# facebookresearch/vilbert-multi-task

Measured on AMD Instinct MI355X. Metric: samples/sec (36 regions, 36 tokens) ViLBERT-base 6L/6C fwd+bwd, higher is better.
Workload: dtype f32; 1 GPU; bert_base_6layer_6conect.json train_concap step: BertForMultiModalPreTraining fwd+bwd (dropout on) + grad all-reduce + AdamW, 36 regions + 1 global row, batch 256 per GPU, T=36 R=37; per_gpu_batch=256, global_batch=256, parallelism=dp1, visible_gpus=1, launch=eager, gemm_mode=f32, deterministic_wgrad=True, deterministic_fallbacks=0

## Files before the change

### vilbert-multi-task_amd/csrc/common.h

```cpp
#pragma once
#include <hip/hip_runtime.h>
#include <stdint.h>

#include "bf16_round.h"
#include "gemm_plan.h"

typedef float f32x4 __attribute__((ext_vector_type(4)));
typedef float f32x16 __attribute__((ext_vector_type(16)));

#define VB_LAUNCH_CHECK()                         \
    do {                                          \
        hipError_t e__ = hipGetLastError();       \
        if (e__ != hipSuccess) return (int)e__;   \
    } while (0)

const uint64_t* vb_seed_epoch();

namespace vbemb {
int text_embed_bwd_det(hipStream_t st, int batch, int n_tok, int hidden, int vocab, int n_types, int n_tasks,
                       const int64_t* ids, const int64_t* seg, const int64_t* task_ids, const float* dx, float* dword,
                       float* dpos, float* dtype, float* dtask);
}

namespace vbrows {
int gather(hipStream_t st, long M, int cols, const float* src, const int32_t* map, long src_rows, float* out);
int drop_add(hipStream_t st, long M, int cols, const float* lin, const float* res, bool res_mapped, const int32_t* map,
             long src_rows, float* out, float p, uint64_t seed);
int invert(hipStream_t st, long src_rows, long M, const int32_t* map, int32_t* inv);
int scatter(hipStream_t st, long src_rows, int cols, const float* compact, const int32_t* inv, float* full);
int scatter_stats(hipStream_t st, long src_rows, const float* v0, const float* v1, const float* v2, const float* v3,
                  const int32_t* inv, float* full);
}

__device__ __forceinline__ float wave_sum(float v) {
#pragma unroll
    for (int off = 32; off > 0; off >>= 1) v += __shfl_xor(v, off, 64);
    return v;
}

__device__ __forceinline__ void gelu_parts(float x, float& phi, float& e) {
    const float z = fabsf(x) * 0.70710678118654752440f;
    const float t = __builtin_amdgcn_rcpf(fmaf(0.3275911f, z, 1.0f));
    e = __expf(-z * z);
    float poly = fmaf(1.061405429f, t, -1.453152027f);
    poly = fmaf(poly, t, 1.421413741f);
    poly = fmaf(poly, t, -0.284496736f);
    poly = fmaf(poly, t, 0.254829592f);
    const float half_erfc = 0.5f * poly * t * e;
    phi = x >= 0.f ? 1.0f - half_erfc : half_erfc;
}

__device__ __forceinline__ float gelu_erf(float x) {
    float phi, e;
    gelu_parts(x, phi, e);
    return x * phi;
}

__device__ __forceinline__ float gelu_grad(float x) {
    float phi, e;
    gelu_parts(x, phi, e);
    return fmaf(x * 0.39894228040143267794f, e, phi);
}

__device__ __forceinline__ void gelu_and_grad(float x, float& y, float& d) {
    float phi, e;
    gelu_parts(x, phi, e);
    y = x * phi;
    d = fmaf(x * 0.39894228040143267794f, e, phi);
}

__device__ __forceinline__ float swish_act(float x) {
    return x / (1.0f + expf(-x));
}

__device__ __forceinline__ float swish_grad(float x) {
    const float s = 1.0f / (1.0f + expf(-x));
    return s + x * s * (1.0f - s);
}
```

### vilbert-multi-task_amd/csrc/layers.hip

```cpp
#include "common.h"
#include "row_map.h"
#include <mutex>
#include <unordered_map>

namespace {

constexpr bool kF32 = false, kB16 = true;

#define VB_TRY(expr)               \
    do {                           \
        const int _e = (expr);     \
        if (_e != 0) return _e;    \
    } while (0)

template <bool B16>
struct Elem { static constexpr size_t size = B16 ? 2 : 4; };

template <bool B16>
inline const void* col(const void* p, long c) { return static_cast<const char*>(p) + c * (long)Elem<B16>::size; }
template <bool B16>
inline void* col(void* p, long c) { return static_cast<char*>(p) + c * (long)Elem<B16>::size; }

bool has_bias(const vb_layer_linear& L) { return L.bias[0] != nullptr; }
bool wants_wgrad(const vb_layer_linear& L) { return L.dw[0] != nullptr; }
// ... 121 lines not shown
        a.mask_add = c.mask; a.O = static_cast<uint16_t*>(c.out); a.ldo = c.ldo; a.lse = c.lse;
        a.scale = scale; a.dropout_p = c.p; a.seed = c.seed;
        return vb_attention_fwd_bf16(st, &a);
    }
    vb_attention_args a{};
    a.batch = c.batch; a.heads = c.heads; a.head_dim = c.d; a.n_q = c.n_q; a.n_k = c.n_k;
    a.q_batch = c.batch; a.kv_batch = c.batch;
    a.Q = static_cast<const float*>(c.q); a.ldq = c.ldq;
    a.K = static_cast<const float*>(c.k); a.ldk = c.ldk;
    a.V = static_cast<const float*>(c.v); a.ldv = c.ldk;
    a.mask_add = c.mask; a.O = static_cast<float*>(c.out); a.ldo = c.ldo; a.lse = c.lse;
    a.scale = scale; a.dropout_p = c.p; a.seed = c.seed;
    return vb_attention_fwd(st, &a);
}

template <bool B16>
int attn_bwd(void* st, const AttnCall& c, const void* d_out, void* dq, void* dk, void* dv, long lddq, long lddk, float* dvec) {
    const float scale = (float)(1.0 / sqrt((double)c.d));
    if (B16) {
        vb_attention_bf16_args a{};
        a.batch = c.batch; a.heads = c.heads; a.head_dim = c.d; a.n_q = c.n_q; a.n_k = c.n_k;
        a.q_batch = c.batch; a.kv_batch = c.batch;
        a.Q = static_cast<const uint16_t*>(c.q); a.ldq = c.ldq;
        a.K = static_cast<const uint16_t*>(c.k); a.ldk = c.ldk;
        a.V = static_cast<const uint16_t*>(c.v); a.ldv = c.ldk;
        a.mask_add = c.mask; a.lse = c.lse; a.scale = scale; a.dropout_p = c.p; a.seed = c.seed;
        vb_attention_bf16_grads g{};
        g.dO = static_cast<const uint16_t*>(d_out); g.lddo = c.ldo;
        g.dQ = static_cast<uint16_t*>(dq); g.lddq = lddq;
        g.dK = static_cast<uint16_t*>(dk); g.lddk = lddk;
        g.dV = static_cast<uint16_t*>(dv); g.lddv = lddk;
        g.dvec = dvec;
        return vb_attention_bwd_bf16(st, &a, &g);
    }
    vb_attention_args a{};
    a.batch = c.batch; a.heads = c.heads; a.head_dim = c.d; a.n_q = c.n_q; a.n_k = c.n_k;
    a.q_batch = c.batch; a.kv_batch = c.batch;
    a.Q = static_cast<const float*>(c.q); a.ldq = c.ldq;
    a.K = static_cast<const float*>(c.k); a.ldk = c.ldk;
    a.V = static_cast<const float*>(c.v); a.ldv = c.ldk;
    a.mask_add = c.mask; a.lse = c.lse; a.scale = scale; a.dropout_p = c.p; a.seed = c.seed;
    vb_attention_grads g{};
    g.dO = static_cast<const float*>(d_out); g.lddo = c.ldo;
    g.dQ = static_cast<float*>(dq); g.lddq = lddq;
    g.dK = static_cast<float*>(dk); g.lddk = lddk;
    g.dV = static_cast<float*>(dv); g.lddv = lddk;
    g.dvec = dvec;
    return vb_attention_bwd(st, &a, &g);
}

std::mutex g_ev_mutex;
std::unordered_map<void*, hipEvent_t> g_fork_events;

int fork_to(void* main_st, void* side_st) {
    hipEvent_t ev;
    {
        std::lock_guard<std::mutex> lock(g_ev_mutex);
        auto it = g_fork_events.find(main_st);
        if (it == g_fork_events.end()) {
            const hipError_t e = hipEventCreateWithFlags(&ev, hipEventDisableTiming);
            if (e != hipSuccess) return (int)e;
            g_fork_events.emplace(main_st, ev);
        } else {
            ev = it->second;
        }
    }
    hipError_t e = hipEventRecord(ev, static_cast<hipStream_t>(main_st));
    if (e != hipSuccess) return (int)e;
    e = hipStreamWaitEvent(static_cast<hipStream_t>(side_st), ev, 0);
    return e == hipSuccess ? 0 : (int)e;
}

struct WgradJob { long M; const vb_layer_linear* L; const void* dY; const void* X; };
struct WgradQueue {
    WgradJob job[8];
    int n = 0;
    void push(long M, const vb_layer_linear& L, const void* dY, const void* X) {
        if (wants_wgrad(L) && n < 8) job[n++] = WgradJob{M, &L, dY, X};
    }
};

template <bool B16>
int wgrad_flush(void* st, void* side, const WgradQueue& q) {
    if (q.n == 0) return 0;
    void* target = st;
    if (side != nullptr && side != st) {
        VB_TRY(fork_to(st, side));
        target = side;
    }
    for (int i = 0; i < q.n; ++i) VB_TRY(wgrad<B16>(target, q.job[i].M, *q.job[i].L, q.job[i].dY, q.job[i].X));
    return 0;
}

AttnCall self_call(const vb_attn_block& b, bool b16) {
    const long Hb = (long)b.heads * b.head_dim, es = b16 ? 2 : 4;
    AttnCall c{};
    c.batch = b.batch; c.heads = b.heads; c.d = b.head_dim; c.n_q = b.n1; c.n_k = b.n1;
    c.q = b.qkv1_out;
    c.k = static_cast<const char*>(b.qkv1_out) + Hb * es;
    c.v = static_cast<const char*>(b.qkv1_out) + 2 * Hb * es;
    c.ldq = c.ldk = 3 * Hb;
    c.mask = b.mask1; c.out = b.ctx1; c.ldo = Hb; c.lse = b.lse1; c.p = b.p1; c.seed = b.seed1;
    return c;
}
AttnCall cross_call(const vb_attn_block& b, bool b16, int which) {
    const long Hb = (long)b.heads * b.head_dim, es = b16 ? 2 : 4;
    const void* qsrc = which == 1 ? b.qkv2_out : b.qkv1_out;
    const void* ksrc = which == 1 ? b.qkv1_out : b.qkv2_out;
    AttnCall c{};
    c.batch = b.batch; c.heads = b.heads; c.d = b.head_dim;
    c.n_q = which == 1 ? b.n2 : b.n1;
    c.n_k = which == 1 ? b.n1 : b.n2;
    c.q = qsrc;
    c.k = static_cast<const char*>(ksrc) + Hb * es;
    c.v = static_cast<const char*>(ksrc) + 2 * Hb * es;
    c.ldq = c.ldk = 3 * Hb;
    c.mask = which == 1 ? b.mask1 : b.mask2;
    c.out = which == 1 ? b.ctx1 : b.ctx2;
    c.ldo = Hb;
    c.lse = which == 1 ? b.lse1 : b.lse2;
    c.p = which == 1 ? b.p1 : b.p2;
    c.seed = which == 1 ? b.seed1 : b.seed2;
    return c;
}

template <bool B16>
int attn_block_fwd(void* st, const vb_attn_block& b) {
    const long M1 = (long)b.batch * b.n1;
    VB_TRY(linear<B16>(st, M1, b.qkv1, b.x1, b.qkv1_out, VB_ACT_NONE, nullptr, 0.f, 0, nullptr));
    if (b.n2 == 0) return attn_fwd<B16>(st, self_call(b, B16));
    const long M2 = (long)b.batch * b.n2;
    VB_TRY(linear<B16>(st, M2, b.qkv2, b.x2, b.qkv2_out, VB_ACT_NONE, nullptr, 0.f, 0, nullptr));
    VB_TRY(attn_fwd<B16>(st, cross_call(b, B16, 1)));
    return attn_fwd<B16>(st, cross_call(b, B16, 2));
}

int ffn_block_rows_fwd(void* st, const vb_ffn_block& f, bool training) {
    hipStream_t hs = static_cast<hipStream_t>(st);
    const long M = f.M, R = f.src_rows;
    float *sum1 = static_cast<float*>(f.sum1), *sum2 = static_cast<float*>(f.sum2);
    VB_TRY(vbrows::gather(hs, M, f.Hc, static_cast<const float*>(f.ctx), f.row_map, R, static_cast<float*>(f.ctx_rows)));
    VB_TRY(linear<kF32>(st, M, f.o, f.ctx_rows, sum1, VB_ACT_NONE, nullptr, 0.f, 0, nullptr));
    VB_TRY(vbrows::drop_add(hs, M, f.H, sum1, static_cast<const float*>(f.x), true, f.row_map, R, sum1, f.p_o, f.seed_o));
    VB_TRY(ln_fwd<kF32>(st, M, f.H, sum1, f.ln1, f.eps, f.a1, training ? f.mean1 : nullptr, training ? f.rstd1 : nullptr));
    VB_TRY(linear<kF32>(st, M, f.f1, f.a1, f.h, VB_ACT_GELU, nullptr, 0.f, 0, training ? f.dact : nullptr));
    VB_TRY(linear<kF32>(st, M, f.f2, f.h, sum2, VB_ACT_NONE, nullptr, 0.f, 0, nullptr));
    VB_TRY(vbrows::drop_add(hs, M, f.H, sum2, static_cast<const float*>(f.a1), false, f.row_map, R, sum2, f.p_f, f.seed_f));
    return ln_fwd<kF32>(st, M, f.H, sum2, f.ln2, f.eps, f.y, training ? f.mean2 : nullptr, training ? f.rstd2 : nullptr);
}

int ffn_block_rows_bwd(void* st, WgradQueue& wq, const vb_ffn_block& f) {
    hipStream_t hs = static_cast<hipStream_t>(st);
    const long M = f.M, R = f.src_rows;
    const vbrows::FullWs w(R, f.H, f.I);
    float* ws = f.full_ws;
    int32_t* inv = reinterpret_cast<int32_t*>(ws + w.inv);
    float* stats = ws + w.stats;
    auto compact = [](const void* p) { return static_cast<const float*>(p); };
    VB_TRY(vbrows::invert(hs, R, M, f.row_map, inv));
    VB_TRY(vbrows::scatter_stats(hs, R, f.mean1, f.rstd1, f.mean2, f.rstd2, inv, stats));
    VB_TRY(vbrows::scatter(hs, R, f.H, compact(f.dy), inv, ws + w.dy));
    VB_TRY(vbrows::scatter(hs, R, f.H, compact(f.sum2), inv, ws + w.sum2));
    VB_TRY(ln_bwd<kF32>(st, R, f.H, ws + w.dy, ws + w.sum2, stats + 2 * R, stats + 3 * R, f.ln2, ws + w.d_sum2, f.ln_ws,
                        ws + w.d_sum2_drop, f.p_f, f.seed_f));
    const float* dyd_full = f.p_f > 0.f ? ws + w.d_sum2_drop : ws + w.d_sum2;
    VB_TRY(vbrows::gather(hs, M, f.H, ws + w.d_sum2, f.row_map, R, static_cast<float*>(f.d_sum2)));
    const void* dyd = f.d_sum2;
    if (f.p_f > 0.f) {
        VB_TRY(vbrows::gather(hs, M, f.H, dyd_full, f.row_map, R, static_cast<float*>(f.d_sum2_drop)));
        dyd = f.d_sum2_drop;
    }
    VB_TRY(dgrad<kF32>(st, M, f.f2, dyd, f.d_pre, nullptr, f.dact));
    VB_TRY(vbrows::scatter(hs, R, f.I, compact(f.h), inv, ws + w.h));
    wq.push(R, f.f2, dyd_full, ws + w.h);
    VB_TRY(dgrad<kF32>(st, M, f.f1, f.d_pre, f.d_a1, f.d_sum2, nullptr));
    VB_TRY(vbrows::scatter(hs, R, f.I, compact(f.d_pre), inv, ws + w.d_pre));
    VB_TRY(vbrows::scatter(hs, R, f.H, compact(f.a1), inv, ws + w.a1));
    wq.push(R, f.f1, ws + w.d_pre, ws + w.a1);
    VB_TRY(vbrows::scatter(hs, R, f.H, compact(f.d_a1), inv, ws + w.d_a1));
    VB_TRY(vbrows::scatter(hs, R, f.H, compact(f.sum1), inv, ws + w.sum1));
    VB_TRY(ln_bwd<kF32>(st, R, f.H, ws + w.d_a1, ws + w.sum1, stats, stats + R, f.ln1, f.d_sum1_full, f.ln_ws,
                        ws + w.d_sum1_drop, f.p_o, f.seed_o));
    const float* dod_full = f.p_o > 0.f ? ws + w.d_sum1_drop : static_cast<const float*>(f.d_sum1_full);
    float* dod = static_cast<float*>(f.p_o > 0.f ? f.d_sum1_drop : f.d_sum1);
    VB_TRY(vbrows::gather(hs, M, f.H, dod_full, f.row_map, R, dod));
    VB_TRY(dgrad<kF32>(st, M, f.o, dod, f.d_ctx, nullptr, nullptr));
    wq.push(R, f.o, dod_full, f.ctx);
    return vbrows::scatter(hs, R, f.Hc, compact(f.d_ctx), inv, static_cast<float*>(f.d_ctx_full));
}

template <bool B16>
int ffn_block_fwd(void* st, const vb_ffn_block& f, bool training) {
    if (f.M == 0) return 0;
    if (f.row_map != nullptr) return ffn_block_rows_fwd(st, f, training);
    VB_TRY(linear<B16>(st, f.M, f.o, f.ctx, f.sum1, VB_ACT_NONE, f.x, f.p_o, f.seed_o, nullptr));
    VB_TRY(ln_fwd<B16>(st, f.M, f.H, f.sum1, f.ln1, f.eps, f.a1, training ? f.mean1 : nullptr, training ? f.rstd1 : nullptr));
    VB_TRY(linear<B16>(st, f.M, f.f1, f.a1, f.h, VB_ACT_GELU, nullptr, 0.f, 0, training ? f.dact : nullptr));
    VB_TRY(linear<B16>(st, f.M, f.f2, f.h, f.sum2, VB_ACT_NONE, f.a1, f.p_f, f.seed_f, nullptr));
    return ln_fwd<B16>(st, f.M, f.H, f.sum2, f.ln2, f.eps, f.y, training ? f.mean2 : nullptr, training ? f.rstd2 : nullptr);
}

template <bool B16>
int ffn_block_bwd(void* st, WgradQueue& wq, const vb_ffn_block& f) {
    if (f.M == 0) return 0;
    if (f.row_map != nullptr) return ffn_block_rows_bwd(st, wq, f);
    VB_TRY(ln_bwd<B16>(st, f.M, f.H, f.dy, f.sum2, f.mean2, f.rstd2, f.ln2, f.d_sum2, f.ln_ws, f.d_sum2_drop, f.p_f, f.seed_f));
    const void* dyd = f.p_f > 0.f ? f.d_sum2_drop : f.d_sum2;
    VB_TRY(dgrad<B16>(st, f.M, f.f2, dyd, f.d_pre, nullptr, f.dact));
    wq.push(f.M, f.f2, dyd, f.h);
    VB_TRY(dgrad<B16>(st, f.M, f.f1, f.d_pre, f.d_a1, f.d_sum2, nullptr));
    wq.push(f.M, f.f1, f.d_pre, f.a1);
    VB_TRY(ln_bwd<B16>(st, f.M, f.H, f.d_a1, f.sum1, f.mean1, f.rstd1, f.ln1, f.d_sum1, f.ln_ws, f.d_sum1_drop, f.p_o, f.seed_o));
    const void* dod = f.p_o > 0.f ? f.d_sum1_drop : f.d_sum1;
    VB_TRY(dgrad<B16>(st, f.M, f.o, dod, f.d_ctx, nullptr, nullptr));
    wq.push(f.M, f.o, dod, f.ctx);
    return 0;
}

template <bool B16>
int attn_block_bwd(void* st, WgradQueue& wq, const vb_attn_block& b) {
    const long Hb = (long)b.heads * b.head_dim, M1 = (long)b.batch * b.n1;
    if (b.n2 == 0) {
        VB_TRY(attn_bwd<B16>(st, self_call(b, B16), b.d_ctx1, b.dqkv1, col<B16>(b.dqkv1, Hb), col<B16>(b.dqkv1, 2 * Hb), 3 * Hb,
                             3 * Hb, b.dvec));
    } else {
        VB_TRY(attn_bwd<B16>(st, cross_call(b, B16, 1), b.d_ctx1, b.dqkv2, col<B16>(b.dqkv1, Hb), col<B16>(b.dqkv1, 2 * Hb), 3 * Hb,
                             3 * Hb, b.dvec));
        VB_TRY(attn_bwd<B16>(st, cross_call(b, B16, 2), b.d_ctx2, b.dqkv1, col<B16>(b.dqkv2, Hb), col<B16>(b.dqkv2, 2 * Hb), 3 * Hb,
                             3 * Hb, b.dvec));
    }
    if (b.dx1 != nullptr) VB_TRY(dgrad<B16>(st, M1, b.qkv1, b.dqkv1, b.dx1, b.dres1, nullptr));
    wq.push(M1, b.qkv1, b.dqkv1, b.x1);
    if (b.n2 != 0) {
        const long M2 = (long)b.batch * b.n2;
        if (b.dx2 != nullptr) VB_TRY(dgrad<B16>(st, M2, b.qkv2, b.dqkv2, b.dx2, b.dres2, nullptr));
        wq.push(M2, b.qkv2, b.dqkv2, b.x2);
    }
    return 0;
}

bool bad_linear(const vb_layer_linear& L, bool b16) {
    if (L.nseg < 1 || L.nseg > VB_MAX_SEGMENTS || L.seg_n <= 0 || L.K <= 0) return true;
    if (b16) return L.w16 == nullptr;
    for (int s = 0; s < L.nseg; ++s)
        if (L.w[s] == nullptr) return true;
    return false;
}

int check(const vb_layer_args* a, bool backward) {
    if (a == nullptr) return VB_E_BADARG;
    if (a->dtype != VB_DT_F32 && a->dtype != VB_DT_BF16) return VB_E_BADARG;
    const bool b16 = a->dtype == VB_DT_BF16;
    const vb_attn_block& b = a->attn;
    const bool has_attn = b.batch != 0;
    if (!has_attn && a->s1.M == 0 && a->s2.M == 0) return VB_E_BADARG;
    if (has_attn) {
        if (b.batch < 0 || b.heads <= 0 || b.head_dim <= 0 || b.n1 <= 0 || b.n2 < 0) return VB_E_BADARG;
        if (b.x1 == nullptr || b.qkv1_out == nullptr || b.ctx1 == nullptr || bad_linear(b.qkv1, b16)) return VB_E_BADARG;
        if ((long)b.qkv1.nseg * b.qkv1.seg_n != 3L * b.heads * b.head_dim) return VB_E_SEGMENT;
        if (b.n2 > 0) {
            if (b.x2 == nullptr || b.qkv2_out == nullptr || b.ctx2 == nullptr || bad_linear(b.qkv2, b16)) return VB_E_BADARG;
            if ((long)b.qkv2.nseg * b.qkv2.seg_n != 3L * b.heads * b.head_dim) return VB_E_SEGMENT;
        }
    }
    for (const vb_ffn_block* f : {&a->s1, &a->s2}) {
        if (f->M == 0) continue;
        if (f->M < 0 || f->H <= 0 || f->I <= 0 || f->Hc <= 0) return VB_E_BADARG;
        if (bad_linear(f->o, b16) || bad_linear(f->f1, b16) || bad_linear(f->f2, b16)) return VB_E_BADARG;
        if (f->o.K != f->Hc || f->o.nseg * f->o.seg_n != f->H || f->f1.K != f->H || f->f1.nseg * f->f1.seg_n != f->I ||
            f->f2.K != f->I || f->f2.nseg * f->f2.seg_n != f->H)
            return VB_E_SEGMENT;
        if (f->ctx == nullptr || f->x == nullptr || f->sum1 == nullptr || f->a1 == nullptr || f->h == nullptr || f->sum2 == nullptr ||
            f->y == nullptr || f->ln1.gamma == nullptr || f->ln2.gamma == nullptr)
            return VB_E_BADARG;
        if (backward) {
            if (f->dy == nullptr || f->d_sum2 == nullptr || f->d_pre == nullptr || f->d_a1 == nullptr || f->d_sum1 == nullptr ||
                f->d_ctx == nullptr || f->ln_ws == nullptr || f->dact == nullptr || f->mean1 == nullptr || f->mean2 == nullptr ||
                f->ln1.dgamma == nullptr || f->ln2.dgamma == nullptr)
                return VB_E_BADARG;
            if ((f->p_f > 0.f && f->d_sum2_drop == nullptr) || (f->p_o > 0.f && f->d_sum1_drop == nullptr)) return VB_E_BADARG;
        }
        if (int e = vbrows::check_row_map(*f, b16, backward)) return e;
    }
    if (backward && has_attn &&
        (b.dqkv1 == nullptr || b.dvec == nullptr || b.d_ctx1 == nullptr || b.lse1 == nullptr ||
         (b.n2 > 0 && (b.dqkv2 == nullptr || b.d_ctx2 == nullptr || b.lse2 == nullptr))))
        return VB_E_BADARG;
    return 0;
}

template <bool B16>
int layer_fwd(void* st, const vb_layer_args* a) {
    if (a->attn.batch != 0) VB_TRY(attn_block_fwd<B16>(st, a->attn));
    VB_TRY(ffn_block_fwd<B16>(st, a->s1, a->training != 0));
    return ffn_block_fwd<B16>(st, a->s2, a->training != 0);
}

template <bool B16>
int layer_bwd(void* st, const vb_layer_args* a) {
    static const bool each = [] { const char* e = getenv("VB_WGRAD_FORK"); return e != nullptr && e[0] == 'e'; }();
    WgradQueue wq;
    VB_TRY(ffn_block_bwd<B16>(st, wq, a->s1));
    if (each) { VB_TRY(wgrad_flush<B16>(st, a->wgrad_stream, wq)); wq.n = 0; }
    VB_TRY(ffn_block_bwd<B16>(st, wq, a->s2));
    if (each) { VB_TRY(wgrad_flush<B16>(st, a->wgrad_stream, wq)); wq.n = 0; }
    if (a->attn.batch != 0) VB_TRY(attn_block_bwd<B16>(st, wq, a->attn));
    return wgrad_flush<B16>(st, a->wgrad_stream, wq);
}

}

extern "C" int vb_layer_fwd(void* stream, const vb_layer_args* a) {
    VB_TRY(check(a, false));
    return a->dtype == VB_DT_BF16 ? layer_fwd<kB16>(stream, a) : layer_fwd<kF32>(stream, a);
}

extern "C" int vb_layer_bwd(void* stream, const vb_layer_args* a) {
    VB_TRY(check(a, true));
    return a->dtype == VB_DT_BF16 ? layer_bwd<kB16>(stream, a) : layer_bwd<kF32>(stream, a);
}
```

### vilbert-multi-task_amd/csrc/rowmap.hip

```cpp
#include "common.h"
#include "rng.h"
#include "row_map.h"

namespace {

__device__ __forceinline__ long source_row(const int32_t* __restrict__ map, long r, long src_rows) {
    const long s = map[r];
    return s >= 0 && s < src_rows ? s : -1;
}

__global__ __launch_bounds__(256) void gather_rows_kernel(long M, int cols4, const f32x4* __restrict__ src,
                                                          const int32_t* __restrict__ map, long src_rows,
                                                          f32x4* __restrict__ out) {
    const long n = M * cols4;
    for (long i = (long)blockIdx.x * blockDim.x + threadIdx.x; i < n; i += (long)gridDim.x * blockDim.x) {
        const long r = i / cols4, c = i - r * cols4;
        const long s = source_row(map, r, src_rows);
        out[i] = s >= 0 ? src[s * cols4 + c] : f32x4{0.f, 0.f, 0.f, 0.f};
    }
}

__global__ __launch_bounds__(256) void row_drop_add_kernel(long M, int cols4, const f32x4* lin, const f32x4* __restrict__ res,
                                                           int res_mapped, const int32_t* __restrict__ map, long src_rows,
                                                           f32x4* out, float p, float scale, uint64_t seed_in,
                                                           const uint64_t* __restrict__ epoch) {
    const uint64_t seed = p > 0.f ? vb_seed_with_epoch(seed_in, epoch) : 0;
    const long n = M * cols4;
    for (long i = (long)blockIdx.x * blockDim.x + threadIdx.x; i < n; i += (long)gridDim.x * blockDim.x) {
        const long r = i / cols4, c = i - r * cols4;
        const long s = source_row(map, r, src_rows);
        f32x4 o = {0.f, 0.f, 0.f, 0.f};
        if (s >= 0) {
            f32x4 v = lin[i];
            if (p > 0.f) {
                const uint64_t idx = (uint64_t)((s * cols4 + c) * 4);
#pragma unroll
                for (int e = 0; e < 4; ++e) v[e] = vb_keep(seed, idx + e, p) ? v[e] * scale : 0.f;
            }
            o = v;
            if (res != nullptr) o += res[(res_mapped ? s : r) * cols4 + c];
        }
        out[i] = o;
    }
}

__global__ __launch_bounds__(256) void invert_map_kernel(long src_rows, int M, const int32_t* __restrict__ map,
                                                         int32_t* __restrict__ inv) {
    const int lane = threadIdx.x & 63;
    const long R = (long)blockIdx.x * 4 + (threadIdx.x >> 6);
    if (R >= src_rows) return;
    int found = -1;
    for (int base = 0; base < M && found < 0; base += 64) {
        const int r = base + lane;
        const unsigned long long hits = __ballot(r < M && (long)map[r] == R);
        if (hits != 0) found = base + __ffsll(hits) - 1;
    }
    if (lane == 0) inv[R] = found;
}

__global__ __launch_bounds__(256) void scatter_rows_kernel(long src_rows, int cols4, const f32x4* __restrict__ compact,
                                                           const int32_t* __restrict__ inv, f32x4* __restrict__ full) {
    const long n = src_rows * cols4;
    for (long i = (long)blockIdx.x * blockDim.x + threadIdx.x; i < n; i += (long)gridDim.x * blockDim.x) {
        const long R = i / cols4, c = i - R * cols4;
        const long r = inv[R];
        full[i] = r >= 0 ? compact[r * cols4 + c] : f32x4{0.f, 0.f, 0.f, 0.f};
    }
}

__global__ __launch_bounds__(256) void scatter_stats_kernel(long src_rows, const float* __restrict__ v0, const float* __restrict__ v1,
                                                            const float* __restrict__ v2, const float* __restrict__ v3,
                                                            const int32_t* __restrict__ inv, float* __restrict__ full) {
    for (long R = (long)blockIdx.x * blockDim.x + threadIdx.x; R < src_rows; R += (long)gridDim.x * blockDim.x) {
        const long r = inv[R];
        full[R] = r >= 0 ? v0[r] : 0.f;
        full[src_rows + R] = r >= 0 ? v1[r] : 0.f;
        full[2 * src_rows + R] = r >= 0 ? v2[r] : 0.f;
        full[3 * src_rows + R] = r >= 0 ? v3[r] : 0.f;
    }
}

inline unsigned grid_for(long work_items) {
    long blocks = (work_items + 255) / 256;
    if (blocks > 2048) blocks = 2048;
    if (blocks < 1) blocks = 1;
    return (unsigned)blocks;
}

}

namespace vbrows {

int gather(hipStream_t st, long M, int cols, const float* src, const int32_t* map, long src_rows, float* out) {
    hipLaunchKernelGGL(gather_rows_kernel, dim3(grid_for(M * (cols / 4))), dim3(256), 0, st, M, cols / 4,
                       reinterpret_cast<const f32x4*>(src), map, src_rows, reinterpret_cast<f32x4*>(out));
    VB_LAUNCH_CHECK();
    return 0;
}

int drop_add(hipStream_t st, long M, int cols, const float* lin, const float* res, bool res_mapped, const int32_t* map,
             long src_rows, float* out, float p, uint64_t seed) {
    hipLaunchKernelGGL(row_drop_add_kernel, dim3(grid_for(M * (cols / 4))), dim3(256), 0, st, M, cols / 4,
                       reinterpret_cast<const f32x4*>(lin), reinterpret_cast<const f32x4*>(res), res_mapped ? 1 : 0, map, src_rows,
                       reinterpret_cast<f32x4*>(out), p, 1.0f / (1.0f - p), seed, p > 0.f ? vb_seed_epoch() : nullptr);
    VB_LAUNCH_CHECK();
    return 0;
}

int invert(hipStream_t st, long src_rows, long M, const int32_t* map, int32_t* inv) {
    hipLaunchKernelGGL(invert_map_kernel, dim3((unsigned)((src_rows + 3) / 4)), dim3(256), 0, st, src_rows, (int)M, map, inv);
    VB_LAUNCH_CHECK();
    return 0;
}

int scatter(hipStream_t st, long src_rows, int cols, const float* compact, const int32_t* inv, float* full) {
    hipLaunchKernelGGL(scatter_rows_kernel, dim3(grid_for(src_rows * (cols / 4))), dim3(256), 0, st, src_rows, cols / 4,
                       reinterpret_cast<const f32x4*>(compact), inv, reinterpret_cast<f32x4*>(full));
    VB_LAUNCH_CHECK();
    return 0;
}

int scatter_stats(hipStream_t st, long src_rows, const float* v0, const float* v1, const float* v2, const float* v3,
                  const int32_t* inv, float* full) {
    hipLaunchKernelGGL(scatter_stats_kernel, dim3(grid_for(src_rows)), dim3(256), 0, st, src_rows, v0, v1, v2, v3, inv, full);
    VB_LAUNCH_CHECK();
    return 0;
}

}
```

### vilbert-multi-task_amd/vilbert/layers.py

```python
import ctypes
import os
import weakref

import torch
from torch.autograd import Function

from . import _native as N
from . import arena as _arena
from . import autograd_ops as A
from . import ops
from . import ops16

BF16 = torch.bfloat16
_STATE = {"on": os.environ.get("VB_LAYER_NATIVE", "1") != "0", "calls": 0}


def set_native(on):
    prev, _STATE["on"] = _STATE["on"], bool(on)
    return prev


def native_calls():
    return _STATE["calls"]

# ... 150 lines not shown
    _static_linear(f.o, [p[0]], [p[1]])
    f.ln1.gamma, f.ln1.beta = p[2].data_ptr(), p[3].data_ptr()
    _static_linear(f.f1, [p[4]], [p[5]])
    _static_linear(f.f2, [p[6]], [p[7]])
    f.ln2.gamma, f.ln2.beta = p[8].data_ptr(), p[9].data_ptr()


def _dyn_ffn_fwd(f, c, base, ctx_ptr, x_ptr, y_ptr, p, dyn, b16, training):
    f.ctx, f.x, f.y = ctx_ptr, x_ptr, y_ptr
    f.p_o, f.p_f, f.seed_o, f.seed_f = dyn
    if b16:
        _shadow_linear(f.o, [p[0]])
        _shadow_linear(f.f1, [p[4]])
        _shadow_linear(f.f2, [p[6]])
    at = c.at
    f.sum1, f.a1, f.h, f.sum2 = at(base, "sum1"), at(base, "a1"), at(base, "h"), at(base, "sum2")
    if training:
        f.dact = at(base, "dact")
        f.mean1, f.rstd1, f.mean2, f.rstd2 = at(base, "mean1"), at(base, "rstd1"), at(base, "mean2"), at(base, "rstd2")


def _dyn_ffn_bwd(f, t, tbase, dy_ptr, d_sum1_ptr, d_ctx_ptr, tg, pbase, ws, dyn):
    p_o, p_f = dyn[0], dyn[1]
    at = t.at
    f.dy = dy_ptr
    f.d_sum2, f.d_pre, f.d_a1 = at(tbase, "d_sum2"), at(tbase, "d_pre"), at(tbase, "d_a1")
    f.d_sum2_drop = at(tbase, "d_sum2_drop") if p_f > 0.0 else None
    f.d_sum1_drop = at(tbase, "d_sum1_drop") if p_o > 0.0 else None
    f.d_sum1, f.d_ctx = d_sum1_ptr, d_ctx_ptr
    f.ln_ws = ws.data_ptr()
    _set_linear_targets(f.o, tg, [pbase + 0], [pbase + 1])
    f.ln1.dgamma, f.ln1.dbeta = tg.overwrite_target(pbase + 2), tg.overwrite_target(pbase + 3)
    _set_linear_targets(f.f1, tg, [pbase + 4], [pbase + 5])
    _set_linear_targets(f.f2, tg, [pbase + 6], [pbase + 7])
    f.ln2.dgamma, f.ln2.dbeta = tg.overwrite_target(pbase + 8), tg.overwrite_target(pbase + 9)


def _ffn_plan(p, dims, b16, training):
    plan = _Plan()
    plan.params, plan.b16, plan.training, plan.dims = list(p), b16, training, dims
    M, _Hc, H, I, _eps = dims
    es = 2 if b16 else 4
    plan.c_fwd = _Carver()
    _ffn_sizes(plan.c_fwd, M, H, I, es, training)
    plan.c_bwd = _Carver()
    _ffn_bwd_sizes(plan.c_bwd, M, H, I, es)
    a = N.LayerArgs()
    a.dtype, a.training = (1 if b16 else 0), int(training)
    _static_ffn(a.s1, p, dims)
    _seal(plan, a)
    return plan


class FfnBlockFn(Function):

    @staticmethod
    def forward(ctx, ctx_t, x, plan, dyn, *p):
        b16, training, c = plan.b16, plan.training, plan.c_fwd
        ctx_t, x = ops._contig(ctx_t), ops._contig(x)
        buf = c.alloc(x.device)
        y = torch.empty_like(x)
        a = plan.new_args()
        _dyn_ffn_fwd(a.s1, c, buf.data_ptr(), ctx_t.data_ptr(), x.data_ptr(), y.data_ptr(), p, dyn, b16, training)
        _call(N.lib().vb_layer_fwd, a, "vb_layer_fwd (output + FFN block)")
        if training:
            ctx.save_for_backward(ctx_t, x, buf, *p)
            ctx.plan, ctx.dyn = plan, dyn
        return y

    @staticmethod
    def backward(ctx, dy):
        ctx_t, x, buf = ctx.saved_tensors[:3]
        p = ctx.saved_tensors[3:]
        plan, dyn = ctx.plan, ctx.dyn
        b16, c, t = plan.b16, plan.c_fwd, plan.c_bwd
        M, _Hc, H, _I, _eps = plan.dims
        dy = ops._contig(dy)
        dev = x.device
        N.ensure_deterministic(dev)
        tg = _Targets(list(p), dev)
        side, ws_stream = _side_stream_for(dev, tg)
        tbuf = t.alloc(dev)
        d_x = torch.empty_like(x)
        d_ctx = torch.empty_like(ctx_t)
        a = plan.new_args()
        a.training, a.wgrad_stream = 1, side
        _dyn_ffn_fwd(a.s1, c, buf.data_ptr(), ctx_t.data_ptr(), x.data_ptr(), buf.data_ptr(), p, dyn, b16, True)
        _dyn_ffn_bwd(a.s1, t, tbuf.data_ptr(), dy.data_ptr(), d_x.data_ptr(), d_ctx.data_ptr(), tg, 0, _ln_ws(dev, M, H, b16), dyn)
        _call(N.lib().vb_layer_bwd, a, "vb_layer_bwd (output + FFN block)")
        if ws_stream is not None:
            for tt in (buf, tbuf, ctx_t, d_x):
                tt.record_stream(ws_stream)
            if dyn[0] == 0.0:
                A.hold_for_side_stream(ws_stream, d_x)
        grads = tg.finish()
        return (d_ctx, d_x, None, None) + tuple(grads)


def _static_attn(b, adims, p):
    b.batch, b.heads, b.head_dim, b.n1, b.n2 = adims
    _static_linear(b.qkv1, [p[0], p[2], p[4]], [p[1], p[3], p[5]])
    if adims[4]:
        _static_linear(b.qkv2, [p[6], p[8], p[10]], [p[7], p[9], p[11]])


def _dyn_attn_fwd(b, n2, x1, x2, mask1, mask2, qkv1, qkv2, ctx1, ctx2, lse1, lse2, p, adyn, b16):
    b.x1, b.mask1, b.qkv1_out, b.ctx1, b.lse1 = x1, mask1, qkv1, ctx1, lse1
    b.p1, b.p2, b.seed1, b.seed2 = adyn
    if b16:
        _shadow_linear(b.qkv1, [p[0], p[2], p[4]])
    if n2:
        b.x2, b.mask2, b.qkv2_out, b.ctx2, b.lse2 = x2, mask2, qkv2, ctx2, lse2
        if b16:
            _shadow_linear(b.qkv2, [p[6], p[8], p[10]])


def _mask2d(mask, B, S):
    if mask is None:
        return None
    m = ops._contig(mask)
    if m.numel() != B * S:
        raise RuntimeError("attention: mask must hold %d x %d values" % (B, S))
    N.dev_f32(m, "attention mask")
    return m


def _ptr(t):
    return t.data_ptr() if t is not None else None


def _self_plan(p, adims, dims, b16, training, row_cap=None):
    plan = _Plan()
    plan.params, plan.b16, plan.training = list(p), b16, training
    plan.dims, plan.row_cap = (adims, dims), row_cap
    B, heads, _d, S, _n2 = adims
    M, _Hc, H, I, _eps = dims
    Mb = M if row_cap is None else row_cap
    es = 2 if b16 else 4
    c = plan.c_fwd = _Carver()
    _ffn_sizes(c, Mb, H, I, es, training)
    c.add("qkv", M * 3 * H * es)
    c.add("ctx", M * H * es)
    if row_cap is not None:
        c.add("ctx_rows", Mb * H * es)
    if training:
        c.add("lse", B * heads * S * 4)
    t = plan.c_bwd = _Carver()
    _ffn_bwd_sizes(t, Mb, H, I, es)
    t.add("d_sum1", M * H * es)
    t.add("d_ctx", M * H * es)
    if row_cap is not None:
        t.add("d_sum1_rows", Mb * H * es)
        t.add("d_ctx_rows", Mb * H * es)
        t.add("full_ws", M * (8 * H + 2 * I + 5) * 4)
    t.add("dqkv", M * 3 * H * es)
    t.add("dvec", B * heads * S * 4)
    a = N.LayerArgs()
    a.dtype, a.training = (1 if b16 else 0), int(training)
    _static_attn(a.attn, adims, p)
    _static_ffn(a.s1, p[6:], dims)
    if row_cap is not None:
        a.s1.src_rows = M
    _seal(plan, a)
    return plan


class SelfLayerFn(Function):

    @staticmethod
    def forward(ctx, x, mask, rows, plan, dyn, *p):
        b16, training, c = plan.b16, plan.training, plan.c_fwd
        (B, _heads, _d, S, _n2), _dims = plan.dims
        x = ops._contig(x)
        mask = _mask2d(mask, B, S)
        buf = c.alloc(x.device)
        base = buf.data_ptr()
        y = torch.empty_like(x) if rows is None else torch.empty((rows.numel(), x.shape[-1]), dtype=x.dtype, device=x.device)
        a = plan.new_args()
        cx = c.at(base, "ctx")
        _dyn_attn_fwd(a.attn, 0, x.data_ptr(), None, _ptr(mask), None, c.at(base, "qkv"), None, cx, None,
                      c.at(base, "lse") if training else None, None, p, (dyn[4], 0.0, dyn[5], 0), b16)
        _dyn_ffn_fwd(a.s1, c, base, cx, x.data_ptr(), y.data_ptr(), p[6:], dyn[:4], b16, training)
        if rows is not None:
            a.s1.M, a.s1.row_map, a.s1.ctx_rows = rows.numel(), rows.data_ptr(), c.at(base, "ctx_rows")
        _call(N.lib().vb_layer_fwd, a, "vb_layer_fwd")
        if training:
            ctx.save_for_backward(x, mask, buf, rows, *p)
            ctx.plan, ctx.dyn = plan, dyn
        return y

    @staticmethod
    def backward(ctx, dy):
        x, mask, buf, rows = ctx.saved_tensors[:4]
        p = ctx.saved_tensors[4:]
        plan, dyn = ctx.plan, ctx.dyn
        b16, c, t = plan.b16, plan.c_fwd, plan.c_bwd
        _adims, (M, _Hc, H, _I, _eps) = plan.dims
        dy = ops._contig(dy)
        dev = x.device
        N.ensure_deterministic(dev)
        tg = _Targets(list(p), dev)
        side, ws_stream = _side_stream_for(dev, tg)
        tbuf = t.alloc(dev)
        base, tbase = buf.data_ptr(), tbuf.data_ptr()
        dx = torch.empty_like(x)
        a = plan.new_args()
        a.training, a.wgrad_stream = 1, side
        cx, d_sum1, d_ctx = c.at(base, "ctx"), t.at(tbase, "d_sum1"), t.at(tbase, "d_ctx")
        _dyn_attn_fwd(a.attn, 0, x.data_ptr(), None, _ptr(mask), None, c.at(base, "qkv"), None, cx, None, c.at(base, "lse"), None,
                      p, (dyn[4], 0.0, dyn[5], 0), b16)
        _dyn_ffn_fwd(a.s1, c, base, cx, x.data_ptr(), c.at(base, "sum1"), p[6:], dyn[:4], b16, True)
        if rows is None:
            _dyn_ffn_bwd(a.s1, t, tbase, dy.data_ptr(), d_sum1, d_ctx, tg, 6, _ln_ws(dev, M, H, b16), dyn)
        else:
            f = a.s1
            _dyn_ffn_bwd(f, t, tbase, dy.data_ptr(), t.at(tbase, "d_sum1_rows"), t.at(tbase, "d_ctx_rows"), tg, 6,
                         _ln_ws(dev, M, H, b16), dyn)
            f.M, f.row_map, f.ctx_rows = rows.numel(), rows.data_ptr(), c.at(base, "ctx_rows")
            f.d_sum1_full, f.d_ctx_full = d_sum1, d_ctx
            f.full_ws = t.at(tbase, "full_ws")
        b = a.attn
        b.d_ctx1, b.dqkv1, b.dvec = d_ctx, t.at(tbase, "dqkv"), t.at(tbase, "dvec")
        b.dres1, b.dx1 = d_sum1, dx.data_ptr()
        _set_linear_targets(b.qkv1, tg, [0, 2, 4], [1, 3, 5])
        _call(N.lib().vb_layer_bwd, a, "vb_layer_bwd")
        if ws_stream is not None:
            for tt in (buf, tbuf, x):
                tt.record_stream(ws_stream)
        grads = tg.finish()
        return (dx, None, None, None, None) + tuple(grads)


def _bi_plan(p, adims, b16, training):
    plan = _Plan()
    plan.params, plan.b16, plan.training, plan.dims = list(p), b16, training, adims
    B, heads, d, n1, n2 = adims
    Hb = heads * d
    es = 2 if b16 else 4
    c = plan.c_fwd = _Carver()
    c.add("qkv1", B * n1 * 3 * Hb * es)
    c.add("qkv2", B * n2 * 3 * Hb * es)
    if training:
        c.add("lse1", B * heads * n2 * 4)
        c.add("lse2", B * heads * n1 * 4)
    t = plan.c_bwd = _Carver()
    t.add("dqkv1", B * n1 * 3 * Hb * es)
    t.add("dqkv2", B * n2 * 3 * Hb * es)
    t.add("dvec", B * heads * max(n1, n2) * 4)
    a = N.LayerArgs()
    a.dtype, a.training = (1 if b16 else 0), int(training)
    _static_attn(a.attn, adims, p)
    _seal(plan, a)
    return plan


class BiAttnBlockFn(Function):

    @staticmethod
    def forward(ctx, x1, x2, mask1, mask2, plan, adyn, *p):
        b16, training, c = plan.b16, plan.training, plan.c_fwd
        B, heads, d, n1, n2 = plan.dims
        Hb = heads * d
        x1, x2 = ops._contig(x1), ops._contig(x2)
        mask1, mask2 = _mask2d(mask1, B, n1), _mask2d(mask2, B, n2)
        buf = c.alloc(x1.device)
        base = buf.data_ptr()
        ctx1 = torch.empty((B, n2, Hb), dtype=x1.dtype, device=x1.device)
        ctx2 = torch.empty((B, n1, Hb), dtype=x1.dtype, device=x1.device)
        a = plan.new_args()
        _dyn_attn_fwd(a.attn, n2, x1.data_ptr(), x2.data_ptr(), _ptr(mask1), _ptr(mask2), c.at(base, "qkv1"), c.at(base, "qkv2"),
                      ctx1.data_ptr(), ctx2.data_ptr(), c.at(base, "lse1") if training else None,
                      c.at(base, "lse2") if training else None, p, adyn, b16)
        _call(N.lib().vb_layer_fwd, a, "vb_layer_fwd (co-attention block)")
        if training:
            ctx.save_for_backward(x1, x2, mask1, mask2, buf, *p)
            ctx.plan, ctx.adyn = plan, adyn
            ctx.set_materialize_grads(False)
        return ctx1, ctx2

    @staticmethod
    def backward(ctx, d1, d2):
        x1, x2, mask1, mask2, buf = ctx.saved_tensors[:5]
        p = ctx.saved_tensors[5:]
        plan, adyn = ctx.plan, ctx.adyn
        if d1 is None and d2 is None:
            return (None,) * (6 + len(p))
        b16, c, t = plan.b16, plan.c_fwd, plan.c_bwd
        B, heads, d, n1, n2 = plan.dims
        Hb = heads * d
        dev = x1.device
        d1 = ops._contig(d1) if d1 is not None else torch.zeros((B, n2, Hb), dtype=x1.dtype, device=dev)
        d2 = ops._contig(d2) if d2 is not None else torch.zeros((B, n1, Hb), dtype=x1.dtype, device=dev)
        N.ensure_deterministic(dev)
        tg = _Targets(list(p), dev)
        side, ws_stream = _side_stream_for(dev, tg)
        tbuf = t.alloc(dev)
        base, tbase = buf.data_ptr(), tbuf.data_ptr()
        dx1, dx2 = torch.empty_like(x1), torch.empty_like(x2)
        a = plan.new_args()
        a.training, a.wgrad_stream = 1, side
        _dyn_attn_fwd(a.attn, n2, x1.data_ptr(), x2.data_ptr(), _ptr(mask1), _ptr(mask2), c.at(base, "qkv1"), c.at(base, "qkv2"),
                      d1.data_ptr(), d2.data_ptr(), c.at(base, "lse1"), c.at(base, "lse2"), p, adyn, b16)
        b = a.attn
        b.d_ctx1, b.d_ctx2 = d1.data_ptr(), d2.data_ptr()
        b.dqkv1, b.dqkv2, b.dvec = t.at(tbase, "dqkv1"), t.at(tbase, "dqkv2"), t.at(tbase, "dvec")
        b.dx1, b.dx2 = dx1.data_ptr(), dx2.data_ptr()
        _set_linear_targets(b.qkv1, tg, [0, 2, 4], [1, 3, 5])
        _set_linear_targets(b.qkv2, tg, [6, 8, 10], [7, 9, 11])
        _call(N.lib().vb_layer_bwd, a, "vb_layer_bwd (co-attention block)")
        if ws_stream is not None:
            for tt in (buf, tbuf, x1, x2):
                tt.record_stream(ws_stream)
        grads = tg.finish()
        return (dx1, dx2, None, None, None, None) + tuple(grads)


def _grad_state(x_list, params):
    if not torch.is_grad_enabled():
        return "infer"
    n_req = 0
    for p in params:
        if p.requires_grad:
            n_req += 1
    if n_req == len(params):
        return "train"
    if n_req == 0 and not any(t.requires_grad for t in x_list):
        return "infer"
    return None


def _dtype_ok(x):
    if not x.is_cuda:
        return False
    if x.dtype == BF16:
        return N.bf16_stream()
    return x.dtype == torch.float32 and not N.fp8_enabled()


def _block_params(dense, ln1, inter, out):
    return [dense.weight, dense.bias, ln1.weight, ln1.bias, inter.dense.weight, inter.dense.bias, out.dense.weight,
            out.dense.bias, out.LayerNorm.weight, out.LayerNorm.bias]


def _block_ok(params, b16, inter_act):
    if inter_act != "gelu" or any(p is None for p in params):
        return False
    if not (_linear_ok([params[0]], [params[1]], b16) and _linear_ok([params[4]], [params[5]], b16)
            and _linear_ok([params[6]], [params[7]], b16)):
        return False
    H = params[2].shape[0]
    return not b16 or (H <= 1024 and H % 4 == 0)


class _NoCtx(object):
    @staticmethod
    def save_for_backward(*a):
        pass


_REFUSED = object()

_SELF_PATHS = ["attention.self.query", "attention.self.key", "attention.self.value", "attention.output.dense",
               "attention.output.LayerNorm", "intermediate.dense", "output.dense", "output.LayerNorm"]
_CONN_PATHS = ["biattention.query1", "biattention.key1", "biattention.value1", "biattention.query2", "biattention.key2",
               "biattention.value2", "biOutput.dense1", "biOutput.LayerNorm1", "v_intermediate.dense", "v_output.dense",
               "v_output.LayerNorm", "biOutput.dense2", "biOutput.LayerNorm2", "t_intermediate.dense", "t_output.dense",
               "t_output.LayerNorm"]


def _wiring(layer, paths):
# ... 181 lines not shown
```

Before: 2565 samples/s.

## Run row-compacted FFN backward on compact rows instead of scattering to full rows

The row-subset FFN backward used to scatter every activation and gradient back to the full source-row space and then run LayerNorm backward and weight-gradient GEMMs over all R rows. It now runs LayerNorm backward and the wgrad pushes directly on the M compact rows, applies dropout masks with drop_add using row_map so the seeds still line up, and scatters only the final d_sum1 and d_ctx back to full rows. This removes many scatter kernels, the stats scatter, and GEMM work on zero rows, and it shrinks the workspace. The cost is a separate dropout-mask pass, and correctness depends on drop_add reproducing the same mask indexing as the fused LN-backward dropout did.

```diff
diff --git a/vilbert-multi-task_amd/csrc/common.h b/vilbert-multi-task_amd/csrc/common.h
--- a/vilbert-multi-task_amd/csrc/common.h
+++ b/vilbert-multi-task_amd/csrc/common.h
@@ -28,8 +28,6 @@
              long src_rows, float* out, float p, uint64_t seed);
 int invert(hipStream_t st, long src_rows, long M, const int32_t* map, int32_t* inv);
 int scatter(hipStream_t st, long src_rows, int cols, const float* compact, const int32_t* inv, float* full);
-int scatter_stats(hipStream_t st, long src_rows, const float* v0, const float* v1, const float* v2, const float* v3,
-                  const int32_t* inv, float* full);
 }
 
 __device__ __forceinline__ float wave_sum(float v) {
diff --git a/vilbert-multi-task_amd/csrc/layers.hip b/vilbert-multi-task_amd/csrc/layers.hip
--- a/vilbert-multi-task_amd/csrc/layers.hip
+++ b/vilbert-multi-task_amd/csrc/layers.hip
@@ -297,40 +297,30 @@
 int ffn_block_rows_bwd(void* st, WgradQueue& wq, const vb_ffn_block& f) {
     hipStream_t hs = static_cast<hipStream_t>(st);
     const long M = f.M, R = f.src_rows;
-    const vbrows::FullWs w(R, f.H, f.I);
-    float* ws = f.full_ws;
-    int32_t* inv = reinterpret_cast<int32_t*>(ws + w.inv);
-    float* stats = ws + w.stats;
+    int32_t* inv = reinterpret_cast<int32_t*>(f.full_ws);
     auto compact = [](const void* p) { return static_cast<const float*>(p); };
-    VB_TRY(vbrows::invert(hs, R, M, f.row_map, inv));
-    VB_TRY(vbrows::scatter_stats(hs, R, f.mean1, f.rstd1, f.mean2, f.rstd2, inv, stats));
-    VB_TRY(vbrows::scatter(hs, R, f.H, compact(f.dy), inv, ws + w.dy));
-    VB_TRY(vbrows::scatter(hs, R, f.H, compact(f.sum2), inv, ws + w.sum2));
-    VB_TRY(ln_bwd<kF32>(st, R, f.H, ws + w.dy, ws + w.sum2, stats + 2 * R, stats + 3 * R, f.ln2, ws + w.d_sum2, f.ln_ws,
-                        ws + w.d_sum2_drop, f.p_f, f.seed_f));
-    const float* dyd_full = f.p_f > 0.f ? ws + w.d_sum2_drop : ws + w.d_sum2;
-    VB_TRY(vbrows::gather(hs, M, f.H, ws + w.d_sum2, f.row_map, R, static_cast<float*>(f.d_sum2)));
+    VB_TRY(ln_bwd<kF32>(st, M, f.H, f.dy, f.sum2, f.mean2, f.rstd2, f.ln2, f.d_sum2, f.ln_ws, nullptr, 0.f, 0));
     const void* dyd = f.d_sum2;
     if (f.p_f > 0.f) {
-        VB_TRY(vbrows::gather(hs, M, f.H, dyd_full, f.row_map, R, static_cast<float*>(f.d_sum2_drop)));
+        VB_TRY(vbrows::drop_add(hs, M, f.H, compact(f.d_sum2), nullptr, false, f.row_map, R, static_cast<float*>(f.d_sum2_drop),
+                                f.p_f, f.seed_f));
         dyd = f.d_sum2_drop;
     }
     VB_TRY(dgrad<kF32>(st, M, f.f2, dyd, f.d_pre, nullptr, f.dact));
-    VB_TRY(vbrows::scatter(hs, R, f.I, compact(f.h), inv, ws + w.h));
-    wq.push(R, f.f2, dyd_full, ws + w.h);
+    wq.push(M, f.f2, dyd, f.h);
     VB_TRY(dgrad<kF32>(st, M, f.f1, f.d_pre, f.d_a1, f.d_sum2, nullptr));
-    VB_TRY(vbrows::scatter(hs, R, f.I, compact(f.d_pre), inv, ws + w.d_pre));
-    VB_TRY(vbrows::scatter(hs, R, f.H, compact(f.a1), inv, ws + w.a1));
-    wq.push(R, f.f1, ws + w.d_pre, ws + w.a1);
-    VB_TRY(vbrows::scatter(hs, R, f.H, compact(f.d_a1), inv, ws + w.d_a1));
-    VB_TRY(vbrows::scatter(hs, R, f.H, compact(f.sum1), inv, ws + w.sum1));
-    VB_TRY(ln_bwd<kF32>(st, R, f.H, ws + w.d_a1, ws + w.sum1, stats, stats + R, f.ln1, f.d_sum1_full, f.ln_ws,
-                        ws + w.d_sum1_drop, f.p_o, f.seed_o));
-    const float* dod_full = f.p_o > 0.f ? ws + w.d_sum1_drop : static_cast<const float*>(f.d_sum1_full);
-    float* dod = static_cast<float*>(f.p_o > 0.f ? f.d_sum1_drop : f.d_sum1);
-    VB_TRY(vbrows::gather(hs, M, f.H, dod_full, f.row_map, R, dod));
+    wq.push(M, f.f1, f.d_pre, f.a1);
+    VB_TRY(ln_bwd<kF32>(st, M, f.H, f.d_a1, f.sum1, f.mean1, f.rstd1, f.ln1, f.d_sum1, f.ln_ws, nullptr, 0.f, 0));
+    const void* dod = f.d_sum1;
+    if (f.p_o > 0.f) {
+        VB_TRY(vbrows::drop_add(hs, M, f.H, compact(f.d_sum1), nullptr, false, f.row_map, R, static_cast<float*>(f.d_sum1_drop),
+                                f.p_o, f.seed_o));
+        dod = f.d_sum1_drop;
+    }
     VB_TRY(dgrad<kF32>(st, M, f.o, dod, f.d_ctx, nullptr, nullptr));
-    wq.push(R, f.o, dod_full, f.ctx);
+    wq.push(M, f.o, dod, f.ctx_rows);
+    VB_TRY(vbrows::invert(hs, R, M, f.row_map, inv));
+    VB_TRY(vbrows::scatter(hs, R, f.H, compact(f.d_sum1), inv, static_cast<float*>(f.d_sum1_full)));
     return vbrows::scatter(hs, R, f.Hc, compact(f.d_ctx), inv, static_cast<float*>(f.d_ctx_full));
 }
 
diff --git a/vilbert-multi-task_amd/csrc/rowmap.hip b/vilbert-multi-task_amd/csrc/rowmap.hip
--- a/vilbert-multi-task_amd/csrc/rowmap.hip
+++ b/vilbert-multi-task_amd/csrc/rowmap.hip
@@ -68,18 +68,6 @@
     }
 }
 
-__global__ __launch_bounds__(256) void scatter_stats_kernel(long src_rows, const float* __restrict__ v0, const float* __restrict__ v1,
-                                                            const float* __restrict__ v2, const float* __restrict__ v3,
-                                                            const int32_t* __restrict__ inv, float* __restrict__ full) {
-    for (long R = (long)blockIdx.x * blockDim.x + threadIdx.x; R < src_rows; R += (long)gridDim.x * blockDim.x) {
-        const long r = inv[R];
-        full[R] = r >= 0 ? v0[r] : 0.f;
-        full[src_rows + R] = r >= 0 ? v1[r] : 0.f;
-        full[2 * src_rows + R] = r >= 0 ? v2[r] : 0.f;
-        full[3 * src_rows + R] = r >= 0 ? v3[r] : 0.f;
-    }
-}
-
 inline unsigned grid_for(long work_items) {
     long blocks = (work_items + 255) / 256;
     if (blocks > 2048) blocks = 2048;
@@ -120,11 +108,4 @@
     return 0;
 }
 
-int scatter_stats(hipStream_t st, long src_rows, const float* v0, const float* v1, const float* v2, const float* v3,
-                  const int32_t* inv, float* full) {
-    hipLaunchKernelGGL(scatter_stats_kernel, dim3(grid_for(src_rows)), dim3(256), 0, st, src_rows, v0, v1, v2, v3, inv, full);
-    VB_LAUNCH_CHECK();
-    return 0;
 }
-
-}
diff --git a/vilbert-multi-task_amd/vilbert/layers.py b/vilbert-multi-task_amd/vilbert/layers.py
--- a/vilbert-multi-task_amd/vilbert/layers.py
+++ b/vilbert-multi-task_amd/vilbert/layers.py
@@ -326,7 +326,7 @@
     if row_cap is not None:
         t.add("d_sum1_rows", Mb * H * es)
         t.add("d_ctx_rows", Mb * H * es)
-        t.add("full_ws", M * (8 * H + 2 * I + 5) * 4)
+        t.add("full_ws", M * 4)
     t.add("dqkv", M * 3 * H * es)
     t.add("dvec", B * heads * S * 4)
     a = N.LayerArgs()
@@ -389,7 +389,7 @@
         else:
             f = a.s1
             _dyn_ffn_bwd(f, t, tbase, dy.data_ptr(), t.at(tbase, "d_sum1_rows"), t.at(tbase, "d_ctx_rows"), tg, 6,
-                         _ln_ws(dev, M, H, b16), dyn)
+                         _ln_ws(dev, max(M, rows.numel()), H, b16), dyn)
             f.M, f.row_map, f.ctx_rows = rows.numel(), rows.data_ptr(), c.at(base, "ctx_rows")
             f.d_sum1_full, f.d_ctx_full = d_sum1, d_ctx
             f.full_ws = t.at(tbase, "full_ws")
```

Measured after the change: 2592 samples/s (median of 6 runs). 1.0% higher.
